# samholt/NeuralLaplaceControl

Hardware: AMD Instinct MI355X
Metric: MPPI planning steps/sec (16384 samples, H=40) (higher is better)
Workload: dtype f64

## Files before the change

### neurallaplacecontrol_amd/csrc/abi_ctx.hip

```cpp
#include "nlc_host.h"

using namespace nlc;
using namespace nlc::host;

namespace nlc {
namespace host {

thread_local std::string g_create_error;

bool gru_use_coop(const nlc_ctx* c, int64_t n_windows) {
  if (c->opt.gru_coop >= 0) return c->opt.gru_coop != 0;
  if (c->g == 128) return true;
  return n_windows <= (c->g == 32 ? 8192 : 50000);
}

void prof_flush(nlc_ctx* c) {
  for (auto& p : c->prof) {
    for (auto& ev : p.pending) {
      hipEventSynchronize(ev.second);
      float ms = 0.f;
      hipEventElapsedTime(&ms, ev.first, ev.second);
      p.total_ms += ms;
      c->event_pool.push_back(ev.first);
      c->event_pool.push_back(ev.second);
// ... 181 lines not shown
  } else if (n == "repfunc_split") {
    if (value != 0 && value != 1) return fail(c, NLC_ERR_BAD_ARG, "repfunc_split must be 0 or 1");
    c->opt.repfunc_split = (int)value;
  } else if (n == "gru_coop") {
    if (value != 0 && value != 1 && value != -1) return fail(c, NLC_ERR_BAD_ARG, "gru_coop must be -1 (auto), 0 or 1");
    c->opt.gru_coop = (int)value;
  } else if (n == "gru_prefix") {
    if (value != 0 && value != 1 && value != -1) return fail(c, NLC_ERR_BAD_ARG, "gru_prefix must be -1 (auto), 0 or 1");
    c->opt.gru_prefix = (int)value;
  } else if (n == "gru_gemm") {
    if (value != 0 && value != 1) return fail(c, NLC_ERR_BAD_ARG, "gru_gemm must be 0 (FP64 MFMA) or 1 (int8-sliced)");
    c->opt.gru_gemm = (int)value;
    if (c->has_model) c->gru.use_i8 = (c->gru.i8_stream != nullptr && value == 1) ? 1 : 0;
  } else if (n == "dbg_gap_us") {
    if (value < 0 || value > 1.0e5) return fail(c, NLC_ERR_BAD_ARG, "dbg_gap_us must be in 0 .. 1e5");
    c->opt.dbg_gap_us = value;
  } else if (n == "dbg_l2_mb") {
    if (value < 0 || value > 4096) return fail(c, NLC_ERR_BAD_ARG, "dbg_l2_mb must be in 0 .. 4096");
    c->opt.dbg_l2_mb = value;
  } else if (n == "fused_max_samples") {
    if (value < 0) return fail(c, NLC_ERR_BAD_ARG, "fused_max_samples must be >= 0");
    c->opt.fused_max_samples = (int64_t)value;
  } else {
    return fail(c, NLC_ERR_BAD_ARG, "unknown option: " + n);
  }
  return NLC_OK;
}

extern "C" int nlc_get_stat(nlc_ctx* c, const char* name, double* out) {
  if (!c) return NLC_ERR_BAD_ARG;
  if (!name || !out) return fail(c, NLC_ERR_BAD_ARG, "NULL stat name / out");
  const std::string n(name);
  if (n == "rollout_body") *out = (double)c->last_body;
  else if (n == "fused_timeouts") *out = (double)c->fused.timeouts;
  else if (n == "fused_fallbacks") *out = (double)c->fused.fallbacks;
  else if (n == "fused_lost") *out = c->fused.lost ? 1.0 : 0.0;
  else if (n == "last_giveup_command") *out = (double)c->fused.last_giveup_command;
  else if (n == "commands") *out = (double)c->commands;
  else if (n == "comm_world") *out = c->comm ? (double)c->comm_world : 0.0;
  else if (n == "comm_rank") *out = c->comm ? (double)c->comm_rank : -1.0;
  else if (n == "fused_blocks_per_cu") *out = (double)c->fused.blocks_per_cu;
  else if (n == "fused_spin_limit") *out = (double)c->opt.fused_spin_limit;
  else if (n == "model_nt3") *out = c->has_model ? (double)c->net.nt3 : 0.0;
  else if (n == "gru_gemm") *out = (c->has_model && c->gru.use_i8) ? 1.0 : 0.0;
  else if (n == "gru_prefix") *out = c->prefix.last_used ? 1.0 : 0.0;
  else if (n.rfind("gru_prefix_windows_l", 0) == 0 && n.size() == 21 && n[20] >= '0' && n[20] <= '4') {
    *out = 0.0;
    if (c->prefix.last_used && c->prefix.lists) {
      unsigned cnt[nlc::prefix::kLists] = {0};
      NLC_HIP(c, hipStreamSynchronize(c->stream));
      NLC_HIP(c, hipMemcpy(cnt, c->prefix.lists, sizeof(cnt), hipMemcpyDeviceToHost));
      *out = (double)cnt[n[20] - '0'];
    }
  } else if (n == "latents_offset") *out = (c->has_mppi && c->pd.dynamics == NLC_DYN_NL) ? (double)ws_layout(c).pa : -1.0;
  else if (n == "gru_i8_launches") *out = (double)nlc::gru_i8_launch_count();
  else return fail(c, NLC_ERR_BAD_ARG, "unknown stat: " + n);
  return NLC_OK;
}

extern "C" int nlc_synchronize(nlc_ctx* c) {
  if (!c) return NLC_ERR_BAD_ARG;
  NLC_HIP(c, hipStreamSynchronize(c->stream));
  return NLC_OK;
}

extern "C" int nlc_device_info(nlc_ctx* c, char* name, int name_len, int* cus, int* mhz, double* gib) {
  if (!c) return NLC_ERR_BAD_ARG;
  if (name && name_len > 0) {
    std::snprintf(name, name_len, "%s (%s)", c->prop.name, c->prop.gcnArchName);
  }
  if (cus) *cus = c->prop.multiProcessorCount;
  if (mhz) *mhz = c->prop.clockRate / 1000;
  if (gib) *gib = (double)c->prop.totalGlobalMem / (1024.0 * 1024.0 * 1024.0);
  return NLC_OK;
}

extern "C" int nlc_profile_enable(nlc_ctx* c, int on) {
  if (!c) return NLC_ERR_BAD_ARG;
  if (!on) prof_flush(c);
  c->profiling = on != 0;
  return NLC_OK;
}
extern "C" int nlc_profile_reset(nlc_ctx* c) {
  if (!c) return NLC_ERR_BAD_ARG;
  prof_flush(c);
  c->prof.clear();
  return NLC_OK;
}
extern "C" int nlc_profile_count(nlc_ctx* c) {
  if (!c) return NLC_ERR_BAD_ARG;
  return (int)c->prof.size();
}
extern "C" int nlc_profile_read(nlc_ctx* c, int idx, char* name, int name_len, double* total_ms, int64_t* launches) {
  if (!c) return NLC_ERR_BAD_ARG;
  if (idx < 0 || idx >= (int)c->prof.size()) return fail(c, NLC_ERR_BAD_ARG, "profile index out of range");
  prof_flush(c);
  const ProfEntry& p = c->prof[idx];
  if (name && name_len > 0) std::snprintf(name, name_len, "%s", p.name.c_str());
  if (total_ms) *total_ms = p.total_ms;
  if (launches) *launches = p.launches;
  return NLC_OK;
}
```

### neurallaplacecontrol_amd/csrc/abi_planner_nl.hip

```cpp
#include "nlc_host.h"

using namespace nlc;
using namespace nlc::host;

namespace {

__global__ void dbg_spin_kernel(unsigned long long ticks_100mhz) {
  const unsigned long long t0 = __builtin_amdgcn_s_memrealtime();
  while (__builtin_amdgcn_s_memrealtime() - t0 < ticks_100mhz) __builtin_amdgcn_s_sleep(8);
}
__global__ void dbg_touch_kernel(const double* __restrict__ p, size_t n, double* __restrict__ sink) {
  double acc = 0.0;
  for (size_t i = (size_t)blockIdx.x * blockDim.x + threadIdx.x; i < n; i += (size_t)gridDim.x * blockDim.x) acc += p[i];
  if (acc == 12345.678) *sink = acc;
}
int dbg_between(nlc_ctx* c) {
  if (c->opt.dbg_gap_us > 0.0) hipLaunchKernelGGL(dbg_spin_kernel, dim3(1), dim3(64), 0, c->stream, (unsigned long long)(c->opt.dbg_gap_us * 100.0));
  if (c->opt.dbg_l2_mb > 0.0) {
    const size_t bytes = (size_t)(c->opt.dbg_l2_mb * 1048576.0);
    const size_t n = bytes / 8 + 1;
    if (c->dbg_scratch_n < n) {
      if (int rc = hold_doubles(c, c->dbg_scratch, n, nullptr, &c->dbg_scratch_n)) return rc;
      NLC_HIP(c, hipMemsetAsync(c->dbg_scratch, 0, n * sizeof(double), c->stream));
    }
// ... 296 lines not shown
  fc.n_enc = s.n_enc;
  fc.roll_cap = s.roll_cap;
  fc.adaptive_q8 = s.adaptive_q8;
  fc.pool_wgs = s.pool_wgs;
  fc.chain_first_tiles = s.chain_first_tiles;
  fc.partner_tiles = s.partner_tiles;
  fc.spin_limit = (unsigned)c->opt.fused_spin_limit;
  fc.test_drop_tile = c->opt.fused_test_drop_tile;
  fc.inline_weights = (c->opt.fused_inline & 1) && d.E == 1 && !d.cost_external;
  fc.inline_perturb = (c->opt.fused_inline & 2) && d.E == 1 && inline_inputs && rng == 1 && d.B <= kFusedMaxInlineB;
  unsigned* sync_words = reinterpret_cast<unsigned*>(ws + w.sync);
  const size_t n_sync = fused_sync_words(d.T, KE);
  if (fc.inline_perturb) {
    if (c->fused.sync_clean_ws != buf->workspace) NLC_HIP(c, hipMemsetAsync(sync_words, 0, n_sync * sizeof(unsigned), c->stream));
  } else {
    p.zero_words = sync_words;
    p.n_zero_words = (int64_t)n_sync;
    if (int rc = launch_shift_perturb(c, call)) return rc;
  }
  c->fused.sync_clean_ws = nullptr;
  c->fused.sync_dirty = true;
  c->fused.last.fused = true;
  c->last_body = 3;
  f.p = p;
  if (fc.inline_weights) f.w = make_weight_args(c, buf);
  {
    ProfScope ps(c, "nl_plan_fused_kernel");
    NLC_HIP(c, launch_nl_plan_fused(f, c->g, s.grid, s.built, c->stream));
  }
  *weights_done = fc.inline_weights != 0;
  return NLC_OK;
}

int gru_prefix_begin(nlc_ctx* c, RolloutCall& call, const GruArgs& g, int64_t N, int chunks, bool* use, GruPrefixArgs* px) {
  *use = false;
  if (c->opt.gru_prefix == 0) return NLC_OK;
  GruPrefixState& ps = c->prefix;
  const char* why = ps.why_not;
  if (!why && ps.last_B != g.B) why = "gru_prefix: the table was built for another action-buffer length";
  if (!why && chunks != 1) why = "gru_prefix: not with the encoder in horizon chunks (horizon_chunks)";
  if (!why && gru_use_coop(c, N)) why = "gru_prefix: this launch takes the cooperative encoder (gru_coop)";
  if (!why && g.use_i8) why = "gru_prefix: the FP64 encoder only (gru_gemm is 1)";
  if (!why) why = prefix::out_of_scope(g.nact, g.nin, 1, g.B, N, true);
  if (why) return c->opt.gru_prefix == 1 ? fail(c, NLC_ERR_UNSUPPORTED, why) : NLC_OK;
  const int64_t stride = (N + 63) / 64 * 64;
  const size_t need = 64 + (size_t)prefix::kLists * (size_t)stride / 2;
  if (need > ps.lists_n) {
    NLC_HIP(c, hipStreamSynchronize(c->stream));
    if (int rc = hold_doubles(c, ps.lists, need, nullptr, &ps.lists_n)) return rc;
  }
  double* base = c->arena.base + ps.arena_off;
  px->table = base;
  px->out_tab = base + (size_t)prefix::kEntries * 2 * c->g;
  px->counts = reinterpret_cast<unsigned*>(ps.lists);
  px->lists = reinterpret_cast<unsigned*>(ps.lists + 64);
  px->list_stride = stride;
  px->img_max = ps.img_max;
  px->img_min = ps.img_min;
  call.p.zero_words = px->counts;
  call.p.n_zero_words = 16;
  *use = true;
  return NLC_OK;
}

int rollout_nl_two_launch(nlc_ctx* c, RolloutCall& call, GruArgs& g, RolloutArgs& r, int variant) {
  const nlc_mppi_desc& d = c->pd;
  const int64_t KE = call.KE;
  bool use_prefix = false;
  GruPrefixArgs px{};
  {
    const int chunks = plan::horizon_chunks((variant != 2 && KE > 8192 && d.E == 1) ? c->opt.horizon_chunks : 1, d.T).C;
    if (int rc = gru_prefix_begin(c, call, g, KE * d.T, chunks, &use_prefix, &px)) return rc;
  }
  if (int rc2 = nlc::host::launch_shift_perturb(c, call)) return rc2;
  const plan::Chunks ck = plan::horizon_chunks((variant != 2 && KE > 8192 && d.E == 1) ? c->opt.horizon_chunks : 1, d.T);
  const int C = ck.C, Tc = ck.Tc;
  if (C == 1) {
    g.t0 = 0;
    g.Tc = d.T;
    g.N = KE * d.T;
    if (use_prefix) {
      {
        ProfScope ps(c, "gru_prefix_index_kernel");
        NLC_HIP(c, launch_gru_prefix_index(g, px, c->stream));
      }
      ProfScope ps(c, "gru_encode_kernel");
      NLC_HIP(c, launch_gru_encode_prefix(g, px, c->g, c->stream));
      c->prefix.last_used = true;
    } else {
      ProfScope ps(c, "gru_encode_kernel");
      NLC_HIP(c, launch_gru_encode(g, c->g, c->stream, gru_use_coop(c, g.N)));
    }
    if (c->opt.dbg_gap_us > 0.0 || c->opt.dbg_l2_mb > 0.0)
      if (int rc3 = dbg_between(c)) return rc3;
    r.t_begin = 0;
    r.t_end = d.T;
    ProfScope ps(c, "nl_rollout_kernel");
    NLC_HIP(c, launch_nl_rollout(r, c->stream, variant));
  } else {
    if (int rc = gru_encode_chunks(c, g, KE, C, Tc, false, 0u)) return rc;
    for (int ch = 0; ch < C; ++ch) {
      r.t_begin = ch * Tc;
      r.t_end = (r.t_begin + Tc <= d.T) ? r.t_begin + Tc : d.T;
      if (r.t_begin >= r.t_end) break;
      NLC_HIP(c, hipStreamWaitEvent(c->stream, c->side.ev_gru[ch], 0));
      ProfScope ps(c, "nl_rollout_kernel");
      NLC_HIP(c, launch_nl_rollout(r, c->stream, 1));
    }
  }
  return NLC_OK;
}

}

int nlc::host::gru_prefix_configure(nlc_ctx* c) {
  const nlc_mppi_desc& d = c->pd;
  GruPrefixState& ps = c->prefix;
  ps.last_B = d.B;
  ps.last_used = false;
  const double img[2] = {prefix::bound_image(d.u_max[0], d.u_scale), prefix::bound_image(d.u_min[0], d.u_scale)};
  bool finite = true;
  for (double v : img) finite = finite && std::isfinite((d.u_scale * v - c->gru.mean[0]) / c->gru.std[0]);
  ps.why_not = prefix::out_of_scope(d.nu, c->md.nin, d.has_bounds, d.B, 0, finite);
  if (ps.why_not) return NLC_OK;
  ps.img_max = prefix::bits_of(img[0]);
  ps.img_min = prefix::bits_of(img[1]);
  std::vector<double> syn((size_t)16 * d.B, 0.0);
  for (int col = 0; col < 16; ++col)
    for (int s = 0; s < prefix::cap(d.B); ++s) syn[(size_t)col * d.B + (d.B - 1 - s)] = img[(col >> s) & 1];
  double* base = c->arena.base + ps.arena_off;
  GruPrefixArgs px{};
  px.table = base;
  px.out_tab = base + (size_t)prefix::kEntries * 2 * c->g;
  double* syn_dev = px.out_tab + 64;
  NLC_HIP(c, hipMemcpy(syn_dev, syn.data(), syn.size() * sizeof(double), hipMemcpyHostToDevice));
  GruArgs a = c->gru;
  a.mode = 1;
  a.perturbed = syn_dev;
  a.abuf = syn_dev;
  a.u_scale = d.u_scale;
  a.T = a.Tc = d.B;
  a.t0 = 0;
  a.Kep = 16;
  a.N = 16;
  a.B = d.B;
  a.nact = 1;
  a.out = nullptr;
  NLC_HIP(c, launch_gru_prefix_table(a, px, c->g, c->stream));
  NLC_HIP(c, hipStreamSynchronize(c->stream));
  return NLC_OK;
}

int nlc::host::rollout_nl(nlc_ctx* c, RolloutCall& call) {
  const nlc_mppi_desc& d = c->pd;
  const nlc_mppi_buffers* buf = call.buf;
  const WsLayout& w = call.w;
  double* ws = call.ws;
  const int64_t KE = call.KE;
  const bool replay = call.replay;
  const bool lin_direct = linear_on_rollout_kernels(c);
  double* pa = ws + w.pa;
  GruArgs g = c->gru;
  g.mode = 1;
  g.perturbed = buf->perturbed;
  g.abuf = call.abuf_dev;
  g.u_scale = d.u_scale;
  g.T = d.T;
  g.B = d.B;
  g.Kep = d.K;
  g.nact = d.nu;
  g.out = pa;
  const SampleCostArgs sc = sample_cost_args(c, call);
  RolloutArgs r{};
  put_sample_cost(r, sc);
  r.Kep = sc.Kep;
  r.net = c->net;
  r.net.b1 = c->b1fold;
  r.B = d.B;
  r.pa = pa;
  r.tn = c->tn;
  r.xcarry = ws + w.xcarry;
  r.ccarry = ws + w.ccarry;
  if (lin_direct) {
    if (!c->cp_lin) return fail(c, NLC_ERR_STATE, "linear-algorithm coefficient tables missing (nlc_mppi_configure)");
    const size_t ng = (size_t)2 * c->net.nt3 * 64;
    r.net.Cp = c->cp_lin;
// ... 43 lines not shown
```

### neurallaplacecontrol_amd/csrc/kernels_gru.hip

```cpp
#include "nlc_device.h"
#include "nlc_gru_prefix.h"
#include "nlc_gru_tile.h"
#include "nlc_kernels.h"

namespace nlc {

template <int G>
__global__ __launch_bounds__(256, G <= 64 ? 2 : 1) void gru_encode_kernel(const GruArgs a) {
  constexpr int KS = G / 4;
  const int lane = threadIdx.x & 63, wave = threadIdx.x >> 6;
  const int q = lane >> 4, c = lane & 15;
  const int64_t w = ((int64_t)blockIdx.x * 4 + wave) * 16 + c;
  const bool valid = w < a.N;
  const int64_t wc = valid ? w : a.N - 1;
  int64_t kk = 0;
  int tt = 0;
  if (a.mode == 1) {
    kk = wc / a.Tc;
    tt = a.t0 + (int)(wc - kk * a.Tc);
  }
  __shared__ double Hs[4][2][KS * 64];
  const double o = gru_encode_tile<G>(a, lane, wc, kk, tt, Hs[wave][0], Hs[wave][1]);
  if (valid && q < 2) {
    const int64_t wo = (a.mode == 1) ? kk * a.T + tt : w;
// ... 15 lines not shown
    int64_t kk = 0;
    int tt = 0;
    if (a.mode == 1) {
      kk = wc / a.Tc;
      tt = a.t0 + (int)(wc - kk * a.Tc);
    }
    const double o = gru_encode_tile_coop<G>(a, lane, wv, wc, kk, tt, Hc);
    if (wv == 0 && valid && q < 2) {
      const int64_t wo = (a.mode == 1) ? kk * a.T + tt : w;
      a.out[wo * 2 + q] = o;
    }
    __syncthreads();
  }
}

hipError_t launch_gru_encode(const GruArgs& a, int g, hipStream_t s, bool coop, unsigned lds_pad_bytes) {
  if (a.N <= 0) return hipSuccess;
  if (g == 64 && a.use_i8 && !coop) return launch_gru_encode_i8(a, s);
  if (coop) {
    const int64_t tiles = (a.N + 15) / 16;
    const dim3 cgrid((unsigned)(tiles < 65536 ? tiles : 65536));
    if (g == 64) {
      hipLaunchKernelGGL(gru_encode_coop_kernel<64>, cgrid, dim3(256), lds_pad_bytes, s, a);
    } else if (g == 32) {
      hipLaunchKernelGGL(gru_encode_coop_kernel<32>, cgrid, dim3(256), lds_pad_bytes, s, a);
    } else if (g == 128) {
      hipLaunchKernelGGL(gru_encode_coop_kernel<128>, cgrid, dim3(256), lds_pad_bytes, s, a);
    } else {
      return hipErrorInvalidValue;
    }
    return hipGetLastError();
  }
  const unsigned grid = (unsigned)((a.N + 63) / 64);
  if (g == 64) {
    hipLaunchKernelGGL((gru_encode_kernel<64>), dim3(grid), dim3(256), 0, s, a);
  } else if (g == 32) {
    hipLaunchKernelGGL((gru_encode_kernel<32>), dim3(grid), dim3(256), 0, s, a);
  } else if (g == 128) {
    hipLaunchKernelGGL((gru_encode_kernel<128>), dim3(grid), dim3(256), 0, s, a);
  } else {
    return hipErrorInvalidValue;
  }
  return hipGetLastError();
}


template <int G>
__global__ __launch_bounds__(64) void gru_prefix_table_kernel(const GruArgs a, const GruPrefixArgs px) {
  constexpr int KS = G / 4;
  const int lane = threadIdx.x & 63;
  const int q = lane >> 4, c = lane & 15;
  __shared__ double Hs[2][KS * 64];
  for (int i = lane; i < 2 * G; i += 64) px.table[i] = 0.0;
  const int steps = prefix::cap(a.B);
  const double o = gru_encode_tile<G, true>(a, lane, c, c, a.B - 1, Hs[0], Hs[1], 0, steps, px.table);
  if (steps == a.B && q < 2 && c < (1 << steps)) px.out_tab[prefix::entry_index(steps, c) * 2 + q] = o;
}

constexpr int kIndexPerThread = 8;
__global__ __launch_bounds__(256) void gru_prefix_index_kernel(const GruArgs a, const GruPrefixArgs px) {
  __shared__ unsigned cnt[8], base[8];
  const int lane = threadIdx.x & 63;
  const int nl = prefix::n_lists(a.B);
  if (threadIdx.x < 8) cnt[threadIdx.x] = 0u;
  __syncthreads();
  const int64_t w0 = (int64_t)blockIdx.x * (256 * kIndexPerThread) + threadIdx.x;
  unsigned cls[kIndexPerThread];
#pragma unroll
  for (int it = 0; it < kIndexPerThread; ++it) {
    const int64_t w = w0 + it * 256;
    int len = 7, pattern = 0;
    if (w < a.N) {
      const int64_t kk = w / a.Tc;
      const int tt = a.t0 + (int)(w - kk * a.Tc);
      const prefix::Class c = prefix::classify(a.perturbed + kk * a.T, tt, a.B, px.img_max, px.img_min);
      len = c.len;
      pattern = c.pattern;
      if (len == a.B) {
        const double* o = px.out_tab + prefix::entry_index(len, pattern) * 2;
        a.out[(kk * a.T + tt) * 2 + 0] = o[0];
        a.out[(kk * a.T + tt) * 2 + 1] = o[1];
      }
    }
    cls[it] = (unsigned)len | ((unsigned)pattern << 3);
    for (int l = 0; l <= prefix::kMaxLen; ++l) {
      const unsigned long long m = __ballot(len == l);
      if (m != 0ull && lane == __ffsll((long long)m) - 1) atomicAdd(&cnt[l], (unsigned)__popcll(m));
    }
  }
  __syncthreads();
  if (threadIdx.x <= prefix::kMaxLen) {
    const unsigned n = cnt[threadIdx.x];
    base[threadIdx.x] = n ? atomicAdd(px.counts + threadIdx.x, n) : 0u;
    cnt[threadIdx.x] = 0u;
  }
  __syncthreads();
#pragma unroll
  for (int it = 0; it < kIndexPerThread; ++it) {
    const int64_t w = w0 + it * 256;
    const int len = (int)(cls[it] & 7u);
    for (int l = 0; l < nl; ++l) {
      const unsigned long long m = __ballot(len == l);
      if (m == 0ull) continue;
      const int leader = __ffsll((long long)m) - 1;
      unsigned b = 0u;
      if (lane == leader) b = atomicAdd(&cnt[l], (unsigned)__popcll(m));
      b = (unsigned)__shfl((int)b, leader);
      if (len == l) {
        const unsigned pos = base[l] + b + (unsigned)__popcll(m & ((1ull << lane) - 1ull));
        if ((int64_t)pos < px.list_stride) px.lists[(int64_t)l * px.list_stride + pos] = (unsigned)w | ((cls[it] >> 3) << prefix::kPatternShift);
      }
    }
  }
}

template <int G>
__global__ __launch_bounds__(256, G <= 64 ? 2 : 1) void gru_encode_prefix_kernel(const GruArgs a, const GruPrefixArgs px) {
  constexpr int KS = G / 4;
  const int lane = threadIdx.x & 63;
  const int wave = __builtin_amdgcn_readfirstlane(threadIdx.x >> 6);
  const int q = lane >> 4, c = lane & 15;
  const int nl = prefix::n_lists(a.B);
  int64_t tile = (int64_t)blockIdx.x * 4 + wave;
  int len = 0;
  unsigned n = 0u;
  for (; len < nl; ++len) {
    n = px.counts[len];
    if ((int64_t)n > px.list_stride) n = (unsigned)px.list_stride;
    const int64_t nt = ((int64_t)n + 15) / 16;
    if (tile < nt) break;
    tile -= nt;
  }
  if (len == nl) return;
  const int64_t idx = tile * 16 + c;
  const bool valid = idx < (int64_t)n;
  const unsigned e = px.lists[(int64_t)len * px.list_stride + (valid ? idx : (int64_t)n - 1)];
  int64_t w = (int64_t)(e & ((1u << prefix::kPatternShift) - 1u));
  if (w >= a.N) w = a.N - 1;
  const int64_t kk = w / a.Tc;
  const int tt = a.t0 + (int)(w - kk * a.Tc);
  __shared__ double Hs[4][2][KS * 64];
  if (len > 0) {
    const int pattern = (int)(e >> prefix::kPatternShift) & ((1 << len) - 1);
    const double* ent = px.table + (size_t)prefix::entry_index(len, pattern) * 2 * G;
#pragma unroll
    for (int ks = 0; ks < KS; ++ks) {
      Hs[wave][0][ks * 64 + lane] = ent[4 * ks + q];
      Hs[wave][1][ks * 64 + lane] = ent[G + 4 * ks + q];
    }
  }
  const double o = gru_encode_tile<G, true>(a, lane, w, kk, tt, Hs[wave][0], Hs[wave][1], len);
  if (valid && q < 2) a.out[(kk * a.T + tt) * 2 + q] = o;
}

hipError_t launch_gru_prefix_table(const GruArgs& a, const GruPrefixArgs& px, int g, hipStream_t s) {
  if (g == 64) {
    hipLaunchKernelGGL(gru_prefix_table_kernel<64>, dim3(1), dim3(64), 0, s, a, px);
  } else if (g == 32) {
    hipLaunchKernelGGL(gru_prefix_table_kernel<32>, dim3(1), dim3(64), 0, s, a, px);
  } else if (g == 128) {
    hipLaunchKernelGGL(gru_prefix_table_kernel<128>, dim3(1), dim3(64), 0, s, a, px);
  } else {
    return hipErrorInvalidValue;
  }
  return hipGetLastError();
}
hipError_t launch_gru_prefix_index(const GruArgs& a, const GruPrefixArgs& px, hipStream_t s) {
  if (a.N <= 0) return hipSuccess;
  const int64_t per_block = 256 * kIndexPerThread;
  hipLaunchKernelGGL(gru_prefix_index_kernel, dim3((unsigned)((a.N + per_block - 1) / per_block)), dim3(256), 0, s, a, px);
  return hipGetLastError();
}
hipError_t launch_gru_encode_prefix(const GruArgs& a, const GruPrefixArgs& px, int g, hipStream_t s) {
  if (a.N <= 0) return hipSuccess;
  const unsigned grid = (unsigned)((prefix::worst_case_tiles(a.N, a.B) + 3) / 4);
  if (g == 64) {
    hipLaunchKernelGGL(gru_encode_prefix_kernel<64>, dim3(grid), dim3(256), 0, s, a, px);
  } else if (g == 32) {
    hipLaunchKernelGGL(gru_encode_prefix_kernel<32>, dim3(grid), dim3(256), 0, s, a, px);
  } else if (g == 128) {
    hipLaunchKernelGGL(gru_encode_prefix_kernel<128>, dim3(grid), dim3(256), 0, s, a, px);
  } else {
    return hipErrorInvalidValue;
  }
  return hipGetLastError();
}

template <int G, int WPB>
__global__ __launch_bounds__(64 * WPB, G <= 64 ? 2 : 1) void rnn_encode_kernel(const RnnArgs a) {
  constexpr int GT = G / 16;
  constexpr int KS = G / 4;
  const int lane = threadIdx.x & 63, wave = threadIdx.x >> 6;
  const int q = lane >> 4, c = lane & 15;
  const int64_t w = ((int64_t)blockIdx.x * WPB + wave) * 16 + c;
  const bool valid = w < a.N;
  const int64_t wc = valid ? w : a.N - 1;
  double in_mean = 0.0, in_std = 1.0;
  if (q < a.nin) {
    in_mean = a.mean[q];
    in_std = a.std[q];
  }
  int64_t kk = 0;
  int tt = 0;
  if (a.mode == 1) {
// ... 69 lines not shown
```

### neurallaplacecontrol_amd/csrc/nlc_gru_prefix.h

```cpp
#pragma once
#include <cstdint>

#if defined(__HIPCC__)
#define NLC_PREFIX_HD __host__ __device__
#else
#define NLC_PREFIX_HD
#endif

namespace nlc {
namespace prefix {

constexpr int kMaxLen = 4;
constexpr int kEntries = (2 << kMaxLen) - 1;
constexpr int kLists = kMaxLen + 1;
constexpr int kMaxB = 32;
constexpr int kPatternShift = 27;
constexpr int64_t kMaxWindows = (int64_t)1 << kPatternShift;

NLC_PREFIX_HD inline uint64_t bits_of(double x) {
  uint64_t u;
  __builtin_memcpy(&u, &x, sizeof(u));
  return u;
}
NLC_PREFIX_HD inline double bound_image(double bound, double u_scale) { return bound / u_scale; }
NLC_PREFIX_HD inline int cap(int B) { return B < kMaxLen ? B : kMaxLen; }
NLC_PREFIX_HD inline int n_lists(int B) { return B < kLists ? B : kLists; }
NLC_PREFIX_HD inline int entry_index(int len, int pattern) { return (1 << len) - 1 + pattern; }

struct Class {
  int len, pattern;
};
NLC_PREFIX_HD inline Class classify(const double* row, int t, int B, uint64_t img_max, uint64_t img_min) {
  Class c{0, 0};
  const int L = cap(B);
  for (int s = 0; s < L; ++s) {
    const int i = t + B - 1 - s;
    if (i < B - 1) break;
    const uint64_t v = bits_of(row[i - (B - 1)]);
    if (v == img_max) {
    } else if (v == img_min) {
      c.pattern |= 1 << s;
    } else {
      break;
    }
    c.len = s + 1;
  }
  return c;
}

NLC_PREFIX_HD inline int64_t worst_case_tiles(int64_t N, int B) { return N / 16 + n_lists(B); }

inline const char* out_of_scope(int nu, int nin, int has_bounds, int B, int64_t N, bool images_finite) {
  if (nu != 1 || nin != 1) return "gru_prefix: one action dimension and no time channel only (nu == nin == 1)";
  if (!has_bounds) return "gru_prefix: the planner has no action bounds";
  if (B > kMaxB) return "gru_prefix: action buffers of up to 32 rows only";
  if (N > kMaxWindows) return "gru_prefix: at most 2^27 windows per launch";
  if (!images_finite) return "gru_prefix: a bound's normalised image is not finite";
  return nullptr;
}

}
}
```

### neurallaplacecontrol_amd/csrc/nlc_gru_tile.h

```cpp
#pragma once
#include "nlc_device.h"
#include "nlc_kernels.h"

namespace nlc {

template <int KS>
__device__ __forceinline__ void chunk_gemm(v4d& c0, v4d& c1, v4d& c2, const double* __restrict__ wc, int lane,
                                           const double* __restrict__ hb) {
  double a_cur[3], a_nxt[3];
  gptr p = opaque(wc);
#pragma unroll
  for (int g = 0; g < 3; ++g) a_cur[g] = p[g * 64 + lane];
  double b_cur = hb[lane], b_nxt = 0.0;
#pragma unroll
  for (int ks = 0; ks < KS; ++ks) {
    if (ks + 1 < KS) {
      p = opaque(p + 3 * 64);
#pragma unroll
      for (int g = 0; g < 3; ++g) a_nxt[g] = p[g * 64 + lane];
      b_nxt = hb[(ks + 1) * 64 + lane];
    }
    c0 = mfma(a_cur[0], b_cur, c0);
    c1 = mfma(a_cur[1], b_cur, c1);
    c2 = mfma(a_cur[2], b_cur, c2);
#pragma unroll
    for (int g = 0; g < 3; ++g) a_cur[g] = a_nxt[g];
    b_cur = b_nxt;
    __builtin_amdgcn_sched_barrier(0);
  }
}

typedef double v2d __attribute__((ext_vector_type(2)));
typedef int v2i __attribute__((ext_vector_type(2)));
__device__ __forceinline__ v2d fma2(v2d a, v2d b, v2d c) { return __builtin_elementwise_fma(a, b, c); }
__device__ __forceinline__ v2d splat2(double x) { return v2d{x, x}; }
__device__ __forceinline__ void exp_ratio2(v2d y, v2d* M, v2d* D) {
  v2d N, sh;
  m::exp_ratio_parts<false>(y, &N, D, &sh);
  *M = v2d{ldexp(N.x, __double2loint(sh.x)), ldexp(N.y, __double2loint(sh.y))};
}
__device__ __forceinline__ double min_neg(double x, double hi) {
  double r;
  asm("v_min_f64 %0, -%1, %2" : "=v"(r) : "v"(x), "s"(hi));
  return r;
}
__device__ __forceinline__ double rcp_refined1(double d) {
  const double r = __builtin_amdgcn_rcp(d);
  const double e = fma(-d, r, 1.0);
  return fma(r, fma(e, e, e), r);
}
__device__ __forceinline__ void sigmoid_parts2(v2d x, v2d* num, v2d* den) {
  v2d M;
  exp_ratio2(v2d{min_neg(x.x, 170.0), min_neg(x.y, 170.0)}, &M, num);
  *den = *num + M;
}
__device__ __forceinline__ void sigmoid_pair2(v2d a, v2d b, v2d* sa, v2d* sb) {
  v2d Da, A, Db, B;
  sigmoid_parts2(a, &Da, &A);
  sigmoid_parts2(b, &Db, &B);
  const v2d P = A * B;
  const double R = rcp_refined1(P.x * P.y);
  const v2d inv = v2d{P.y, P.x} * splat2(R);
  *sa = (Da * B) * inv;
  *sb = (Db * A) * inv;
}
__device__ __forceinline__ v2d tanh2(v2d x) {
  const v2d mx = v2d{m::min_abs(x.x, 372.5), m::min_abs(x.y, 372.5)};
  v2d N, D, sh;
  m::exp_ratio_parts<true>(-mx, &N, &D, &sh);
  const v2d M = v2d{ldexp(N.x, __double2loint(sh.x)), ldexp(N.y, __double2loint(sh.y))};
  const v2d num = D - M, d = D + M;
  const double R = rcp_refined1(d.x * d.y);
  const v2d t = (num * v2d{d.y, d.x}) * splat2(R);
  return __builtin_elementwise_copysign(t, x);
}

__device__ __forceinline__ double nan_if_bad_window(bool bad_input, double value) {
  int bad = bad_input ? 1 : 0;
  bad |= __shfl_xor(bad, 16);
  bad |= __shfl_xor(bad, 32);
  return bad ? __builtin_nan("") : value;
}

__device__ __forceinline__ v4d gru_gates(const v4d& ar, const v4d& az, const v4d& ain, const v4d& ahn, const v4d& hold) {
  v4d hnew;
#pragma unroll
  for (int half = 0; half < 2; ++half) {
    const v2d r2 = half ? ar.zw : ar.xy, z2 = half ? az.zw : az.xy, in2 = half ? ain.zw : ain.xy;
    const v2d hn2 = half ? ahn.zw : ahn.xy, ho2 = half ? hold.zw : hold.xy;
    v2d rg, zg;
    sigmoid_pair2(r2, z2, &rg, &zg);
    const v2d ng = tanh2(fma2(rg, hn2, in2));
    const v2d hv = fma2(zg, ho2 - ng, ng);
    if (half) {
      hnew.zw = hv;
    } else {
      hnew.xy = hv;
    }
  }
  return hnew;
}

template <int G, bool kPrefix = false>
__device__ __forceinline__ double gru_encode_tile(const GruArgs& a, int lane, int64_t wc, int64_t kk, int tt,
                                                  double* __restrict__ H0, double* __restrict__ H1, int s0 = 0,
                                                  int s_end = -1, double* __restrict__ dump = nullptr) {
  constexpr int GT = G / 16;
  constexpr int KS = G / 4;
  const int q = lane >> 4;
  double in_mean = 0.0, in_std = 1.0;
  if (q < a.nin) {
    in_mean = a.mean[q];
    in_std = a.std[q];
  }
  const int ab_off = (a.mode == 1) ? (int)(kk / a.Kep) * a.B : 0;
  if (!kPrefix || s0 == 0) {
#pragma unroll
    for (int ks = 0; ks < KS; ++ks) {
      H0[ks * 64 + lane] = 0.0;
      H1[ks * 64 + lane] = 0.0;
    }
  }
  v4d hn[GT];
  bool bad_input = false;

  for (int s = kPrefix ? s0 : 0; s < ((kPrefix && s_end >= 0) ? s_end : a.B); ++s) {
    const int j_win = a.B - 1 - s;
    double xin = 0.0;
    if (q < a.nin) {
      double raw;
      if (a.mode == 0) {
        raw = a.window[(wc * a.B + j_win) * a.nin + q];
      } else {
        const int i = tt + j_win;
        if (q < a.nact)
          raw = (i < a.B - 1) ? a.abuf[(ab_off + 1 + i) * a.nact + q]
                              : a.u_scale * a.perturbed[(kk * a.T + (i - (a.B - 1))) * a.nact + q];
        else
          raw = (double)(a.B - 1 - j_win);
      }
      xin = (raw - in_mean) / in_std;
      bad_input = bad_input || !(xin - xin == 0.0);
    } else if (q == 3) {
      xin = 1.0;
    }
#pragma unroll
    for (int j = 0; j < GT; ++j) {
      gptr wp = opaque(a.Wih0p + (size_t)j * 3 * 64);
      v4d ar = mfma(wp[lane], xin, splat(0.0));
      v4d az = mfma(wp[64 + lane], xin, splat(0.0));
      v4d ain = mfma(wp[128 + lane], xin, splat(0.0));
      v4d ahn = load_bias_tile(a.bhn0, j, q);
      if (s > 0) chunk_gemm<KS>(ar, az, ahn, a.Whh0p + (size_t)j * KS * 3 * 64, lane, H0);
      const v4d hold = {H0[(4 * j + 0) * 64 + lane], H0[(4 * j + 1) * 64 + lane], H0[(4 * j + 2) * 64 + lane],
                        H0[(4 * j + 3) * 64 + lane]};
      hn[j] = gru_gates(ar, az, ain, ahn, hold);
    }
#pragma unroll
    for (int j = 0; j < GT; ++j)
#pragma unroll
      for (int r = 0; r < 4; ++r) H0[(4 * j + r) * 64 + lane] = hn[j][r];
#pragma unroll
    for (int j = 0; j < GT; ++j) {
      v4d ar = load_bias_tile(a.brz1, j, q);
      v4d az = load_bias_tile(a.brz1, GT + j, q);
      v4d ain = load_bias_tile(a.bin1, j, q);
      v4d ahn = load_bias_tile(a.bhn1, j, q);
      chunk_gemm<KS>(ar, az, ain, a.Wih1p + (size_t)j * KS * 3 * 64, lane, H0);
      if (s > 0) chunk_gemm<KS>(ar, az, ahn, a.Whh1p + (size_t)j * KS * 3 * 64, lane, H1);
      const v4d hold = {H1[(4 * j + 0) * 64 + lane], H1[(4 * j + 1) * 64 + lane], H1[(4 * j + 2) * 64 + lane],
                        H1[(4 * j + 3) * 64 + lane]};
      hn[j] = gru_gates(ar, az, ain, ahn, hold);
    }
#pragma unroll
    for (int j = 0; j < GT; ++j)
#pragma unroll
      for (int r = 0; r < 4; ++r) H1[(4 * j + r) * 64 + lane] = hn[j][r];
    if (kPrefix && dump != nullptr && (lane & 15) < (2 << s)) {
      double* e = dump + (size_t)((2 << s) - 1 + (lane & 15)) * 2 * G;
#pragma unroll
      for (int ks = 0; ks < KS; ++ks) {
        e[4 * ks + q] = H0[ks * 64 + lane];
        e[G + 4 * ks + q] = H1[ks * 64 + lane];
      }
    }
  }
  v4d o[1];
  o[0] = splat(0.0);
  gemm_acc<1, KS>(o, a.Wop, lane, [&](int ks) { return H1[ks * 64 + lane]; });
  return nan_if_bad_window(bad_input, o[0][0] + a.bo[q < 2 ? q : 0]);
}

struct XDirect {
  __device__ __forceinline__ void prepare(const GruArgs&, int, int, int64_t, int, bool) {}
  __device__ __forceinline__ double raw(const GruArgs& a, int64_t wc, int64_t kk, int tt, int j_win, int q, int c,
                                        int ab_off) const {
    if (a.mode == 0) return a.window[(wc * a.B + j_win) * a.nin + q];
    const int i = tt + j_win;
    if (q < a.nact)
      return (i < a.B - 1) ? a.abuf[(ab_off + 1 + i) * a.nact + q]
                           : a.u_scale * a.perturbed[(kk * a.T + (i - (a.B - 1))) * a.nact + q];
    return (double)(a.B - 1 - j_win);
  }
};

template <int G, class XS = XDirect>
__device__ __forceinline__ double gru_encode_tile_coop(const GruArgs& a, int lane, int wv, int64_t wc, int64_t kk, int tt,
                                                       double* __restrict__ Hc, XS xs = XS(), bool valid = true) {
  constexpr int GT = G / 16;
  constexpr int KS = G / 4;
  constexpr int CPW = (GT + 3) / 4;
  constexpr bool kAllWaves = GT % 4 == 0;
  constexpr int IMG = KS * 64;
  const int q = lane >> 4;
  double in_mean = 0.0, in_std = 1.0;
  if (q < a.nin) {
    in_mean = a.mean[q];
    in_std = a.std[q];
  }
  const int ab_off = (a.mode == 1) ? (int)(kk / a.Kep) * a.B : 0;
  xs.prepare(a, lane, wv, kk, tt, valid);
#pragma unroll
  for (int i = 0; i < CPW; ++i) {
    const int j = wv + 4 * i;
    if (kAllWaves || j < GT) {
#pragma unroll
      for (int r = 0; r < 4; ++r) {
        Hc[(4 * j + r) * 64 + lane] = 0.0;
        Hc[2 * IMG + (4 * j + r) * 64 + lane] = 0.0;
      }
    }
  }
  __syncthreads();
  bool bad_input = false;
  for (int s = 0; s < a.B; ++s) {
    const int cur = s & 1, nxt = cur ^ 1;
    double* H0c = Hc + cur * IMG;
    double* H0n = Hc + nxt * IMG;
    double* H1c = Hc + (2 + cur) * IMG;
    double* H1n = Hc + (2 + nxt) * IMG;
    const int j_win = a.B - 1 - s;
    double xin = 0.0;
    if (q < a.nin) {
      const double raw = xs.raw(a, wc, kk, tt, j_win, q, lane & 15, ab_off);
      xin = (raw - in_mean) / in_std;
      bad_input = bad_input || !(xin - xin == 0.0);
    } else if (q == 3) {
      xin = 1.0;
    }
#pragma unroll
    for (int i = 0; i < CPW; ++i) {
      const int j = wv + 4 * i;
      if (kAllWaves || j < GT) {
        gptr wp = opaque(a.Wih0p + (size_t)j * 3 * 64);
        v4d ar = mfma(wp[lane], xin, splat(0.0));
        v4d az = mfma(wp[64 + lane], xin, splat(0.0));
        v4d ain = mfma(wp[128 + lane], xin, splat(0.0));
        v4d ahn = load_bias_tile(a.bhn0, j, q);
        if (s > 0) chunk_gemm<KS>(ar, az, ahn, a.Whh0p + (size_t)j * KS * 3 * 64, lane, H0c);
        const v4d hold = {H0c[(4 * j + 0) * 64 + lane], H0c[(4 * j + 1) * 64 + lane], H0c[(4 * j + 2) * 64 + lane],
                          H0c[(4 * j + 3) * 64 + lane]};
        const v4d hn = gru_gates(ar, az, ain, ahn, hold);
#pragma unroll
        for (int r = 0; r < 4; ++r) H0n[(4 * j + r) * 64 + lane] = hn[r];
      }
    }
    __syncthreads();
#pragma unroll
    for (int i = 0; i < CPW; ++i) {
      const int j = wv + 4 * i;
      if (kAllWaves || j < GT) {
        v4d ar = load_bias_tile(a.brz1, j, q);
        v4d az = load_bias_tile(a.brz1, GT + j, q);
        v4d ain = load_bias_tile(a.bin1, j, q);
        v4d ahn = load_bias_tile(a.bhn1, j, q);
        chunk_gemm<KS>(ar, az, ain, a.Wih1p + (size_t)j * KS * 3 * 64, lane, H0n);
        if (s > 0) chunk_gemm<KS>(ar, az, ahn, a.Whh1p + (size_t)j * KS * 3 * 64, lane, H1c);
        const v4d hold = {H1c[(4 * j + 0) * 64 + lane], H1c[(4 * j + 1) * 64 + lane], H1c[(4 * j + 2) * 64 + lane],
                          H1c[(4 * j + 3) * 64 + lane]};
        const v4d hn = gru_gates(ar, az, ain, ahn, hold);
#pragma unroll
        for (int r = 0; r < 4; ++r) H1n[(4 * j + r) * 64 + lane] = hn[r];
      }
    }
  }
  __syncthreads();
  double out = 0.0;
  if (wv == 0) {
    const double* Hl = Hc + (2 + (a.B & 1)) * IMG;
    v4d o[1];
    o[0] = splat(0.0);
    gemm_acc<1, KS>(o, a.Wop, lane, [&](int ks) { return Hl[ks * 64 + lane]; });
    out = o[0][0] + a.bo[q < 2 ? q : 0];
  }
  return nan_if_bad_window(bad_input, out);
}

}
```

### neurallaplacecontrol_amd/csrc/nlc_host.h

```cpp
#pragma once
#include <dlfcn.h>
#include <hip/hip_runtime.h>

#include <time.h>

#include <cmath>
#include <cstdio>
#include <cstdlib>
#include <cstring>
#include <stdexcept>
#include <string>
#include <vector>

#include "nlc_gru_prefix.h"
#include "nlc_kernels.h"
#include "nlc_pack.h"
#include "nlc_plan.h"

namespace nlc {
int nl_pick_nt3(int need);

namespace host {

struct ProfEntry {
// ... 325 lines not shown

struct Rccl {
  typedef struct { char internal[NLC_COMM_ID_BYTES]; } UniqueId;
  int (*GetUniqueId)(UniqueId*) = nullptr;
  int (*CommInitRank)(void**, int, UniqueId, int) = nullptr;
  int (*CommDestroy)(void*) = nullptr;
  int (*AllGather)(const void*, void*, size_t, int, void*, hipStream_t) = nullptr;
  const char* (*GetErrorString)(int) = nullptr;
  std::string why;
  bool ok = false;
};
Rccl* rccl();
constexpr int kNcclFloat64 = 8;

bool linear_on_rollout_kernels(const nlc_ctx* c);
struct WsLayout {
  size_t tile_part, chunk_part, pa, state0, abuf, xcarry, ccarry, fre, fim, dx, tconst, rq, sync, total;
};
WsLayout ws_layout(const nlc_ctx* c);
inline unsigned* pin_giveup_word(nlc_ctx* c) { return reinterpret_cast<unsigned*>(c->pinned + c->pin.giveup); }
inline unsigned long long* pin_seq_word(nlc_ctx* c) { return reinterpret_cast<unsigned long long*>(c->pinned + c->pin.seq); }
inline unsigned* pin_merge_status_word(nlc_ctx* c) { return reinterpret_cast<unsigned*>(c->pinned + c->pin.merge_status); }
WeightArgs make_weight_args(nlc_ctx* c, const nlc_mppi_buffers* buf);
int run_weights(nlc_ctx* c, const nlc_mppi_buffers* buf);
inline int cost_variant_of(const nlc_mppi_desc& d) {
  if (d.cost_external || !(d.cost_variant & (NLC_COST_STATE_CONSTRAINT | NLC_COST_CHANGE_GOAL))) return 0;
  return d.cost_variant;
}
template <class A>
void cost_in_body(A& a, const nlc_mppi_desc& d) {
  if (cost_variant_of(d)) {
    a.env = d.env;
    a.cost_variant = cost_variant_of(d);
  }
}
int finish_rollout_costs(nlc_ctx* c, const nlc_mppi_buffers* buf, bool in_body = false);

struct RolloutCall {
  const nlc_mppi_buffers* buf;
  PerturbArgs p;
  WsLayout w;
  double* ws;
  double* state_dev;
  double* abuf_dev;
  int64_t KE;
  int state_per_sample, rng;
  bool inline_inputs;
  bool replay;
};
int launch_shift_perturb(nlc_ctx* c, RolloutCall& call);
SampleCostArgs sample_cost_args(const nlc_ctx* c, const RolloutCall& call);
int rollout_nl(nlc_ctx* c, RolloutCall& call);
int gru_prefix_configure(nlc_ctx* c);
inline size_t gru_prefix_arena_doubles(int g) {
  return (size_t)nlc::prefix::kEntries * 2 * g + 64 + (size_t)16 * nlc::prefix::kMaxB;
}

}
}
```

### neurallaplacecontrol_amd/csrc/nlc_kernels.h

```cpp
#pragma once
#include <hip/hip_runtime.h>
#include <stdint.h>

#include <climits>
#include <type_traits>

#include "../../include/nlc.h"
#include "nlc_ilt_tile.h"

namespace nlc {

struct IltArgs {
  const double* theta;
  const double* phi;
  const double* t;
  double* x;
  int64_t N;
  int d, S;
  double alpha, log_tol, scale;
  const double* fre;
  const double* fim;
  double t_div;
  int t_stride;
  int rpp, iters;
// ... 52 lines not shown
  int64_t N;
  int d, S;
  const double* wr;
  const double* wi;
};
hipError_t launch_ilt_linear_bwd(const IltLinBwdArgs& a, hipStream_t s);
struct IltDehoogBwdArgs {
  const double* theta;
  const double* phi;
  const double* t;
  const double* gx;
  double* gtheta;
  double* gphi;
  int64_t N;
  int d, S;
  double alpha, log_tol, scale, t_div;
  void* scratch;
};
int64_t ilt_dehoog_bwd_scratch_bytes(int64_t N, int d, int S, unsigned* grid_out);
hipError_t launch_ilt_dehoog_bwd(const IltDehoogBwdArgs& a, hipStream_t s);

struct GruArgs {
  const double* window;
  const double* perturbed;
  const double* abuf;
  double u_scale;
  int mode, T;
  int t0, Tc;
  int64_t Kep;
  int64_t N;
  int B, nin;
  int nact;
  double mean[NLC_MAX_NIN], std[NLC_MAX_NIN];
  const double* Wih0p;
  const double* Whh0p;
  const double* Wih1p;
  const double* Whh1p;
  const double* Wop;
  const double* bhn0;
  const double* brz1;
  const double* bin1;
  const double* bhn1;
  double bo[2];
  double* out;
  int use_i8;
  const signed char* i8_stream;
};
hipError_t launch_gru_encode(const GruArgs& a, int g, hipStream_t s, bool coop = false, unsigned lds_pad_bytes = 0);
hipError_t launch_gru_encode_i8(const GruArgs& a, hipStream_t s);
unsigned long long gru_i8_launch_count();
struct GruPrefixArgs {
  double* table;
  double* out_tab;
  unsigned* lists;
  unsigned* counts;
  int64_t list_stride;
  unsigned long long img_max, img_min;
};
hipError_t launch_gru_prefix_table(const GruArgs& a, const GruPrefixArgs& px, int g, hipStream_t s);
hipError_t launch_gru_prefix_index(const GruArgs& a, const GruPrefixArgs& px, hipStream_t s);
hipError_t launch_gru_encode_prefix(const GruArgs& a, const GruPrefixArgs& px, int g, hipStream_t s);

struct SampleCostArgs {
  int64_t K;
  int64_t Kep;
  int T;
  int nu;
  int env;
  int state_per_sample;
  const double* state0;
  const double* perturbed;
  const double* noise;
  const double* U;
  double sigma_inv[NLC_MAX_NU * NLC_MAX_NU];
  double lambda_;
  double u_scale;
  int noise_abs_cost;
  double* states;
  double* cost_total;
  SampleCostArgs part(int64_t o, int64_t n, int d) const {
    SampleCostArgs v = *this;
    v.K = n;
    if (n < K) v.Kep = n;
    v.state0 = state0 + (state_per_sample ? o * d : 0);
    v.perturbed = perturbed + o * T * nu;
    v.noise = noise + o * T * nu;
    v.states = states ? states + o * T * d : nullptr;
    v.cost_total = cost_total + o;
    return v;
  }
};

struct RnnArgs {
  const double* window;
  const double* perturbed;
  const double* abuf;
  double u_scale;
  int mode, T;
  int64_t Kep;
  int64_t K;
  int64_t N;
  int B, nin, d;
  double mean[NLC_MAX_NIN], std[NLC_MAX_NIN];
  const double* Wihp;
  const double* Whhp;
  const double* bhn;
// ... 380 lines not shown
```

Baseline: 260.7.

## Cache recurrent-gate products in GRU prefix table to skip first resumed step's hidden GEMMs

```diff
diff --git a/neurallaplacecontrol_amd/csrc/abi_ctx.hip b/neurallaplacecontrol_amd/csrc/abi_ctx.hip
--- a/neurallaplacecontrol_amd/csrc/abi_ctx.hip
+++ b/neurallaplacecontrol_amd/csrc/abi_ctx.hip
@@ -257,6 +257,14 @@
       NLC_HIP(c, hipMemcpy(cnt, c->prefix.lists, sizeof(cnt), hipMemcpyDeviceToHost));
       *out = (double)cnt[n[20] - '0'];
     }
+  } else if (n == "gru_prefix_table_tiles") {
+    *out = 0.0;
+    if (c->prefix.last_used && c->prefix.lists) {
+      unsigned cnt[nlc::prefix::kLists] = {0};
+      NLC_HIP(c, hipStreamSynchronize(c->stream));
+      NLC_HIP(c, hipMemcpy(cnt, c->prefix.lists, sizeof(cnt), hipMemcpyDeviceToHost));
+      for (int l = 1; l < nlc::prefix::n_lists(c->prefix.last_B); ++l) *out += (double)((cnt[l] + 15u) / 16u);
+    }
   } else if (n == "latents_offset") *out = (c->has_mppi && c->pd.dynamics == NLC_DYN_NL) ? (double)ws_layout(c).pa : -1.0;
   else if (n == "gru_i8_launches") *out = (double)nlc::gru_i8_launch_count();
   else return fail(c, NLC_ERR_BAD_ARG, "unknown stat: " + n);
diff --git a/neurallaplacecontrol_amd/csrc/abi_planner_nl.hip b/neurallaplacecontrol_amd/csrc/abi_planner_nl.hip
--- a/neurallaplacecontrol_amd/csrc/abi_planner_nl.hip
+++ b/neurallaplacecontrol_amd/csrc/abi_planner_nl.hip
@@ -372,6 +372,7 @@
   double* base = c->arena.base + ps.arena_off;
   px->table = base;
   px->out_tab = base + (size_t)prefix::kEntries * 2 * c->g;
+  px->products = base + gru_prefix_products_off(c->g);
   px->counts = reinterpret_cast<unsigned*>(ps.lists);
   px->lists = reinterpret_cast<unsigned*>(ps.lists + 64);
   px->list_stride = stride;
@@ -452,6 +453,7 @@
   GruPrefixArgs px{};
   px.table = base;
   px.out_tab = base + (size_t)prefix::kEntries * 2 * c->g;
+  px.products = base + gru_prefix_products_off(c->g);
   double* syn_dev = px.out_tab + 64;
   NLC_HIP(c, hipMemcpy(syn_dev, syn.data(), syn.size() * sizeof(double), hipMemcpyHostToDevice));
   GruArgs a = c->gru;
diff --git a/neurallaplacecontrol_amd/csrc/kernels_gru.hip b/neurallaplacecontrol_amd/csrc/kernels_gru.hip
--- a/neurallaplacecontrol_amd/csrc/kernels_gru.hip
+++ b/neurallaplacecontrol_amd/csrc/kernels_gru.hip
@@ -91,9 +91,10 @@
   const int q = lane >> 4, c = lane & 15;
   __shared__ double Hs[2][KS * 64];
   for (int i = lane; i < 2 * G; i += 64) px.table[i] = 0.0;
-  const int steps = prefix::cap(a.B);
-  const double o = gru_encode_tile<G, true>(a, lane, c, c, a.B - 1, Hs[0], Hs[1], 0, steps, px.table);
-  if (steps == a.B && q < 2 && c < (1 << steps)) px.out_tab[prefix::entry_index(steps, c) * 2 + q] = o;
+  const int steps = prefix::build_steps(a.B);
+  const double o = gru_encode_tile<G, kTileBuildTable>(a, lane, c, c, a.B - 1, Hs[0], Hs[1], 0, steps, px.table,
+                                                       px.products - px.table);
+  if (a.B <= prefix::kMaxLen && q < 2 && c < (1 << a.B)) px.out_tab[prefix::entry_index(a.B, c) * 2 + q] = o;
 }
 
 constexpr int kIndexPerThread = 8;
@@ -179,16 +180,19 @@
   const int64_t kk = w / a.Tc;
   const int tt = a.t0 + (int)(w - kk * a.Tc);
   __shared__ double Hs[4][2][KS * 64];
+  double* prod = nullptr;
   if (len > 0) {
     const int pattern = (int)(e >> prefix::kPatternShift) & ((1 << len) - 1);
-    const double* ent = px.table + (size_t)prefix::entry_index(len, pattern) * 2 * G;
+    const int entry = prefix::entry_index(len, pattern);
+    const double* ent = px.table + (size_t)entry * 2 * G;
+    prod = px.products + prefix::products_entry_offset(entry, G);
 #pragma unroll
     for (int ks = 0; ks < KS; ++ks) {
       Hs[wave][0][ks * 64 + lane] = ent[4 * ks + q];
       Hs[wave][1][ks * 64 + lane] = ent[G + 4 * ks + q];
     }
   }
-  const double o = gru_encode_tile<G, true>(a, lane, w, kk, tt, Hs[wave][0], Hs[wave][1], len);
+  const double o = gru_encode_tile<G, kTileFromTable>(a, lane, w, kk, tt, Hs[wave][0], Hs[wave][1], len, -1, prod);
   if (valid && q < 2) a.out[(kk * a.T + tt) * 2 + q] = o;
 }
 
diff --git a/neurallaplacecontrol_amd/csrc/nlc_gru_prefix.h b/neurallaplacecontrol_amd/csrc/nlc_gru_prefix.h
--- a/neurallaplacecontrol_amd/csrc/nlc_gru_prefix.h
+++ b/neurallaplacecontrol_amd/csrc/nlc_gru_prefix.h
@@ -48,6 +48,14 @@
   return c;
 }
 
+NLC_PREFIX_HD inline bool starts_tile(int len, int B) { return len >= 1 && len < n_lists(B); }
+NLC_PREFIX_HD inline int build_steps(int B) { return B <= kMaxLen ? B : kMaxLen + 1; }
+NLC_PREFIX_HD inline int64_t products_doubles(int g) { return (int64_t)(kEntries - 1) * 6 * g; }
+NLC_PREFIX_HD inline int64_t products_entry_offset(int entry, int g) { return (int64_t)(entry - 1) * 6 * g; }
+NLC_PREFIX_HD inline int products_index(int layer, int j, int set, int q, int r, int g) {
+  return (((layer * (g / 16) + j) * 3 + set) * 4 + q) * 4 + r;
+}
+
 NLC_PREFIX_HD inline int64_t worst_case_tiles(int64_t N, int B) { return N / 16 + n_lists(B); }
 
 inline const char* out_of_scope(int nu, int nin, int has_bounds, int B, int64_t N, bool images_finite) {
diff --git a/neurallaplacecontrol_amd/csrc/nlc_gru_tile.h b/neurallaplacecontrol_amd/csrc/nlc_gru_tile.h
--- a/neurallaplacecontrol_amd/csrc/nlc_gru_tile.h
+++ b/neurallaplacecontrol_amd/csrc/nlc_gru_tile.h
@@ -1,5 +1,6 @@
 #pragma once
 #include "nlc_device.h"
+#include "nlc_gru_prefix.h"
 #include "nlc_kernels.h"
 
 namespace nlc {
@@ -101,10 +102,12 @@
   return hnew;
 }
 
-template <int G, bool kPrefix = false>
+enum { kTileFull = 0, kTileFromTable = 1, kTileBuildTable = 2 };
+template <int G, int kMode = kTileFull>
 __device__ __forceinline__ double gru_encode_tile(const GruArgs& a, int lane, int64_t wc, int64_t kk, int tt,
                                                   double* __restrict__ H0, double* __restrict__ H1, int s0 = 0,
-                                                  int s_end = -1, double* __restrict__ dump = nullptr) {
+                                                  int s_end = -1, double* __restrict__ tab = nullptr,
+                                                  int64_t tab_products = 0) {
   constexpr int GT = G / 16;
   constexpr int KS = G / 4;
   const int q = lane >> 4;
@@ -114,7 +117,7 @@
     in_std = a.std[q];
   }
   const int ab_off = (a.mode == 1) ? (int)(kk / a.Kep) * a.B : 0;
-  if (!kPrefix || s0 == 0) {
+  if (kMode != kTileFromTable || s0 == 0) {
 #pragma unroll
     for (int ks = 0; ks < KS; ++ks) {
       H0[ks * 64 + lane] = 0.0;
@@ -124,7 +127,8 @@
   v4d hn[GT];
   bool bad_input = false;
 
-  for (int s = kPrefix ? s0 : 0; s < ((kPrefix && s_end >= 0) ? s_end : a.B); ++s) {
+  auto step = [&](int s, auto tab_c) __attribute__((always_inline)) {
+    constexpr bool kTab = decltype(tab_c)::value;
     const int j_win = a.B - 1 - s;
     double xin = 0.0;
     if (q < a.nin) {
@@ -144,14 +148,39 @@
     } else if (q == 3) {
       xin = 1.0;
     }
+    auto tab_set = [&](int l, int j, int set) -> v4d* {
+      return reinterpret_cast<v4d*>(tab + prefix::products_index(l, j, set, q, 0, G));
+    };
+    double* put = nullptr;
+    if (kMode == kTileBuildTable && s > 0 && (lane & 15) < (1 << s))
+      put = tab + tab_products + prefix::products_entry_offset(prefix::entry_index(s, lane & 15), G);
+    auto put_sets = [&](int l, int j, const v4d& ar, const v4d& az, const v4d& ahn) {
+      if (put == nullptr) return;
+#pragma unroll
+      for (int r = 0; r < 4; ++r) {
+        put[prefix::products_index(l, j, 0, q, r, G)] = ar[r];
+        put[prefix::products_index(l, j, 1, q, r, G)] = az[r];
+        put[prefix::products_index(l, j, 2, q, r, G)] = ahn[r];
+      }
+    };
 #pragma unroll
     for (int j = 0; j < GT; ++j) {
       gptr wp = opaque(a.Wih0p + (size_t)j * 3 * 64);
-      v4d ar = mfma(wp[lane], xin, splat(0.0));
-      v4d az = mfma(wp[64 + lane], xin, splat(0.0));
-      v4d ain = mfma(wp[128 + lane], xin, splat(0.0));
-      v4d ahn = load_bias_tile(a.bhn0, j, q);
-      if (s > 0) chunk_gemm<KS>(ar, az, ahn, a.Whh0p + (size_t)j * KS * 3 * 64, lane, H0);
+      v4d ar, az, ahn;
+      if (kTab) {
+        ar = *tab_set(0, j, 0);
+        az = *tab_set(0, j, 1);
+        ahn = *tab_set(0, j, 2);
+      } else {
+        ar = splat(0.0);
+        az = splat(0.0);
+        ahn = load_bias_tile(a.bhn0, j, q);
+        if (s > 0) chunk_gemm<KS>(ar, az, ahn, a.Whh0p + (size_t)j * KS * 3 * 64, lane, H0);
+        if (kMode == kTileBuildTable) put_sets(0, j, ar, az, ahn);
+      }
+      ar = mfma(wp[lane], xin, ar);
+      az = mfma(wp[64 + lane], xin, az);
+      const v4d ain = mfma(wp[128 + lane], xin, splat(0.0));
       const v4d hold = {H0[(4 * j + 0) * 64 + lane], H0[(4 * j + 1) * 64 + lane], H0[(4 * j + 2) * 64 + lane],
                         H0[(4 * j + 3) * 64 + lane]};
       hn[j] = gru_gates(ar, az, ain, ahn, hold);
@@ -162,12 +191,20 @@
       for (int r = 0; r < 4; ++r) H0[(4 * j + r) * 64 + lane] = hn[j][r];
 #pragma unroll
     for (int j = 0; j < GT; ++j) {
-      v4d ar = load_bias_tile(a.brz1, j, q);
-      v4d az = load_bias_tile(a.brz1, GT + j, q);
+      v4d ar, az, ahn;
+      if (kTab) {
+        ar = *tab_set(1, j, 0);
+        az = *tab_set(1, j, 1);
+        ahn = *tab_set(1, j, 2);
+      } else {
+        ar = load_bias_tile(a.brz1, j, q);
+        az = load_bias_tile(a.brz1, GT + j, q);
+        ahn = load_bias_tile(a.bhn1, j, q);
+        if (s > 0) chunk_gemm<KS>(ar, az, ahn, a.Whh1p + (size_t)j * KS * 3 * 64, lane, H1);
+        if (kMode == kTileBuildTable) put_sets(1, j, ar, az, ahn);
+      }
       v4d ain = load_bias_tile(a.bin1, j, q);
-      v4d ahn = load_bias_tile(a.bhn1, j, q);
       chunk_gemm<KS>(ar, az, ain, a.Wih1p + (size_t)j * KS * 3 * 64, lane, H0);
-      if (s > 0) chunk_gemm<KS>(ar, az, ahn, a.Whh1p + (size_t)j * KS * 3 * 64, lane, H1);
       const v4d hold = {H1[(4 * j + 0) * 64 + lane], H1[(4 * j + 1) * 64 + lane], H1[(4 * j + 2) * 64 + lane],
                         H1[(4 * j + 3) * 64 + lane]};
       hn[j] = gru_gates(ar, az, ain, ahn, hold);
@@ -176,15 +213,22 @@
     for (int j = 0; j < GT; ++j)
 #pragma unroll
       for (int r = 0; r < 4; ++r) H1[(4 * j + r) * 64 + lane] = hn[j][r];
-    if (kPrefix && dump != nullptr && (lane & 15) < (2 << s)) {
-      double* e = dump + (size_t)((2 << s) - 1 + (lane & 15)) * 2 * G;
+    if (kMode == kTileBuildTable && s < prefix::kMaxLen && (lane & 15) < (2 << s)) {
+      double* e = tab + (size_t)((2 << s) - 1 + (lane & 15)) * 2 * G;
 #pragma unroll
       for (int ks = 0; ks < KS; ++ks) {
         e[4 * ks + q] = H0[ks * 64 + lane];
         e[G + 4 * ks + q] = H1[ks * 64 + lane];
       }
     }
-  }
+  };
+
+  int s = (kMode == kTileFromTable) ? s0 : 0;
+  if (kMode == kTileFromTable && s0 > 0) {
+    step(s, std::true_type{});
+    ++s;
+  }
+  for (const int end = (kMode == kTileBuildTable) ? s_end : a.B; s < end; ++s) step(s, std::false_type{});
   v4d o[1];
   o[0] = splat(0.0);
   gemm_acc<1, KS>(o, a.Wop, lane, [&](int ks) { return H1[ks * 64 + lane]; });
@@ -253,11 +297,12 @@
       const int j = wv + 4 * i;
       if (kAllWaves || j < GT) {
         gptr wp = opaque(a.Wih0p + (size_t)j * 3 * 64);
-        v4d ar = mfma(wp[lane], xin, splat(0.0));
-        v4d az = mfma(wp[64 + lane], xin, splat(0.0));
-        v4d ain = mfma(wp[128 + lane], xin, splat(0.0));
+        v4d ar = splat(0.0), az = splat(0.0);
         v4d ahn = load_bias_tile(a.bhn0, j, q);
         if (s > 0) chunk_gemm<KS>(ar, az, ahn, a.Whh0p + (size_t)j * KS * 3 * 64, lane, H0c);
+        ar = mfma(wp[lane], xin, ar);
+        az = mfma(wp[64 + lane], xin, az);
+        const v4d ain = mfma(wp[128 + lane], xin, splat(0.0));
         const v4d hold = {H0c[(4 * j + 0) * 64 + lane], H0c[(4 * j + 1) * 64 + lane], H0c[(4 * j + 2) * 64 + lane],
                           H0c[(4 * j + 3) * 64 + lane]};
         const v4d hn = gru_gates(ar, az, ain, ahn, hold);
@@ -274,8 +319,8 @@
         v4d az = load_bias_tile(a.brz1, GT + j, q);
         v4d ain = load_bias_tile(a.bin1, j, q);
         v4d ahn = load_bias_tile(a.bhn1, j, q);
+        if (s > 0) chunk_gemm<KS>(ar, az, ahn, a.Whh1p + (size_t)j * KS * 3 * 64, lane, H1c);
         chunk_gemm<KS>(ar, az, ain, a.Wih1p + (size_t)j * KS * 3 * 64, lane, H0n);
-        if (s > 0) chunk_gemm<KS>(ar, az, ahn, a.Whh1p + (size_t)j * KS * 3 * 64, lane, H1c);
         const v4d hold = {H1c[(4 * j + 0) * 64 + lane], H1c[(4 * j + 1) * 64 + lane], H1c[(4 * j + 2) * 64 + lane],
                           H1c[(4 * j + 3) * 64 + lane]};
         const v4d hn = gru_gates(ar, az, ain, ahn, hold);
diff --git a/neurallaplacecontrol_amd/csrc/nlc_host.h b/neurallaplacecontrol_amd/csrc/nlc_host.h
--- a/neurallaplacecontrol_amd/csrc/nlc_host.h
+++ b/neurallaplacecontrol_amd/csrc/nlc_host.h
@@ -401,9 +401,10 @@
 SampleCostArgs sample_cost_args(const nlc_ctx* c, const RolloutCall& call);
 int rollout_nl(nlc_ctx* c, RolloutCall& call);
 int gru_prefix_configure(nlc_ctx* c);
+inline size_t gru_prefix_products_off(int g) { return (size_t)nlc::prefix::kEntries * 2 * g + 64 + (size_t)16 * nlc::prefix::kMaxB; }
 inline size_t gru_prefix_arena_doubles(int g) {
-  return (size_t)nlc::prefix::kEntries * 2 * g + 64 + (size_t)16 * nlc::prefix::kMaxB;
-}
-
-}
-}
+  return gru_prefix_products_off(g) + (size_t)nlc::prefix::products_doubles(g);
+}
+
+}
+}
diff --git a/neurallaplacecontrol_amd/csrc/nlc_kernels.h b/neurallaplacecontrol_amd/csrc/nlc_kernels.h
--- a/neurallaplacecontrol_amd/csrc/nlc_kernels.h
+++ b/neurallaplacecontrol_amd/csrc/nlc_kernels.h
@@ -128,6 +128,7 @@
 struct GruPrefixArgs {
   double* table;
   double* out_tab;
+  double* products;
   unsigned* lists;
   unsigned* counts;
   int64_t list_stride;
```

New measurement: 272.1 (median of 6 runs). 1.04x the previous value.
